# StefanHeng/Symbolic-Music-Generation

Hardware: AMD Instinct MI355X
Metric: train tokens/sec (TransfoXL seq2048 bf16), whole job (higher is better)
Workload: dtype bf16; 1 GPU; TransfoXL 12L/768d H12 dh64 F3072 T=2048 M=2048 V=1190 cutoffs=[] (SURVEY C3, mode R: fresh zero mems); per_gpu_batch=64, global_batch=64, seq_len=2048, mem_len=2048, parallelism=dp1

## Files before the change

### include/musicxl.h

```cpp
#ifndef MUSICXL_H
#define MUSICXL_H

#ifdef __cplusplus
extern "C" {
#endif

#define MXL_ABI_VERSION 2

int mxl_abi_version(void);
const char* mxl_error_string(int code);

#define MXL_GEMM_OUT_F32        0x01
#define MXL_GEMM_OUT_F32_ATOMIC 0x02
#define MXL_GEMM_BIAS           0x04
#define MXL_GEMM_RELU           0x08
#define MXL_GEMM_DROPOUT        0x10
#define MXL_GEMM_RELU_BWD       0x20
#define MXL_GEMM_ADD_AUX        0x40
int mxl_set_reserved_cus(int k);
int mxl_gemm_last_nt_kernel(void);

#define MXL_GEMM_SAVE_RELU_MASK 0x100
#define MXL_GEMM_RELU_BWD_BITS  0x200
size_t mxl_gemm_relu_mask_bytes(int M, int N);
// ... 44 lines not shown
                              long long q_bs, int q_rs, long long kv_bs, int kv_rs, int rd_rs, long long o_bs, int o_rs,
                              long long dq_bs, int dq_rs, long long dkv_bs, int dkv_rs, float scale, void* stream);
int mxl_relattn_fwd_phantom(const void* q, const void* k, const void* v, const void* rd, const float* r_w_bias,
                            const float* r_r_bias, void* out, float* lse, void* oph, float* mph, int B, int T, int H,
                            int dh, int M, int Kc, long long q_bs, int q_rs, long long kv_bs, int kv_rs, int rd_rs,
                            long long o_bs, int o_rs, float scale, void* stream);
int mxl_relattn_bwd_sparse_dg_oph(const void* q, const void* k, const void* v, const void* rd, const float* r_w_bias,
                                  const float* r_r_bias, const void* out, const void* dout, const float* lse,
                                  float* delta, void* dq, void* dk, void* dv, void* dg, float* d_r_w_bias,
                                  const void* oph, const float* mph, int B, int T, int H, int dh, int M, int Kc,
                                  long long q_bs, int q_rs, long long kv_bs, int kv_rs, int rd_rs, long long o_bs, int o_rs,
                                  long long dq_bs, int dq_rs, long long dkv_bs, int dkv_rs, float scale, void* stream);
int mxl_relattn_drd_recompute(const void* dg, const void* qr, float* d_rd, int B, int T, int H, int dh, int M, long long qr_bs,
                              int qr_rs, int drd_ld, const void* rd, int rd_rs, float* d_r_r_bias, float* d_r_w_bias_fix,
                              const float* lse, const float* delta, float scale, int Kc, void* stream);

size_t mxl_relattn_bwd_fused_ws_bytes(int B, int T, int H, int dh, int M);
int mxl_relattn_bwd_fused(const void* q, const void* k, const void* v, const void* rd, const float* r_w_bias,
                          const float* r_r_bias, const void* out, const void* dout, const float* lse, float* delta,
                          void* dq, void* dk, void* dv, float* d_rd, int drd_ld, float* d_r_w_bias, float* d_r_r_bias,
                          const void* oph, const float* mph, void* ws, int B, int T, int H, int dh, int M, int Kc,
                          long long q_bs, int q_rs, long long kv_bs, int kv_rs, int rd_rs, long long o_bs, int o_rs,
                          long long dq_bs, int dq_rs, long long dkv_bs, int dkv_rs, float scale, int defer_finish, void* stream);
int mxl_relattn_dq_finish(const void* ws, const void* oph, const float* mph, const float* lse, const float* delta, void* dq,
                          float* d_r_r_bias, int B, int T, int H, int dh, int M, int Kc, long long o_bs, int o_rs, long long dq_bs,
                          int dq_rs, float scale, void* stream);
int mxl_relattn_fwd_phantom2(const void* q, const void* k, const void* v, const void* rd, const float* r_w_bias,
                             const float* r_r_bias, void* out, float* lse, void* oph, float* mph, int oph_all, void* ph_ws, int B,
                             int T, int H, int dh, int M, int Kc, long long q_bs, int q_rs, long long kv_bs, int kv_rs, int rd_rs,
                             long long o_bs, int o_rs, float scale, void* stream);
size_t mxl_relattn_drd_phantom_ws_bytes(int B, int T, int H);
int mxl_relattn_drd_phantom_prep(const void* q, long long q_bs, int q_rs, const float* r_r_bias, const float* lse, void* ws, int B, int T,
                                 int H, int dh, float scale, void* stream);
int mxl_relattn_drd_phantom(const void* ws, const float* delta, float* d_rd, int B, int T, int H, int dh, int M, int drd_ld,
                            const void* rd, int rd_rs, int Kc, void* stream);

int mxl_sinusoid_table(void* out, int M, int d, int clamp_len, float drop_p, unsigned long long seed, unsigned site,
                       void* stream);
int mxl_embed_fwd(const void* ids, const void* E, void* out, int N, int d, int V, float scale, float drop_p,
                  unsigned long long seed, unsigned site, void* stream);
int mxl_embed_bwd(const void* ids, const void* dout, const void* dout2, float* dE, int N, int d, int V, float scale,
                  float drop_p, unsigned long long seed, unsigned site, void* stream);
int mxl_dropout_bf16(const void* x, void* y, long long n, float drop_p, unsigned long long seed, unsigned site,
                     void* stream);
int mxl_ln_residual_fwd(const void* x, const void* res, const float* gamma, const float* beta, void* y, void* z,
                        float* mean, float* rstd, int N, int d, float eps, float drop_p, unsigned long long seed,
// ... 211 lines not shown
```

### symbolic_music_generation_amd/csrc/musicxl_internal.h

```cpp
#pragma once
#include <hip/hip_runtime.h>
#include "../../include/musicxl.h"

namespace mxl_kt {
extern int g_on;
void begin(int id, hipStream_t s);
void end(int id, hipStream_t s);
struct Scope {
    int id; hipStream_t s; bool on;
    Scope(int id_, hipStream_t s_) : id(id_), s(s_), on(g_on != 0) { if (on) begin(id, s); }
    ~Scope() { if (on) end(id, s); }
};
}
```

### symbolic_music_generation_amd/csrc/relattn_bwd_fused.hip

```cpp
#include <cstdlib>
#include <type_traits>
#include "common.h"
#include "musicxl_internal.h"

namespace {

typedef __attribute__((ext_vector_type(8))) __bf16 mfma_bf16x8;
typedef __attribute__((address_space(3))) bf16x4 lds_bf16x4;
typedef _Float16 f16x4 __attribute__((ext_vector_type(4)));
typedef float f32x4v __attribute__((ext_vector_type(4)));

#ifndef FUSED_PF
#define FUSED_PF 3
#endif
#ifndef FUSED_VF_RELOAD
#define FUSED_VF_RELOAD 0
#endif
#ifndef FUSED_PARK
#define FUSED_PARK 0
#endif
#ifndef FUSED_SB
#define FUSED_SB 1
#endif
#define UNIT_FENCE() do { if (FUSED_SB) __builtin_amdgcn_sched_barrier(0); } while (0)
// ... 37 lines not shown
#define STAMP(i) { unsigned long long t_; __builtin_amdgcn_sched_barrier(0); asm volatile("s_memtime %0\n\ts_waitcnt lgkmcnt(0)" : "=s"(t_) :: "memory"); \
    __builtin_amdgcn_sched_barrier(0); st_acc[i] += t_ - st_last; st_last = t_; }
#define STAMP_FLUSH if ((threadIdx.x & 63) == 0) { for (int i_ = 0; i_ < 16; i_++) atomicAdd(&g_fused_stamps[i_], st_acc[i_]); }
#else
#define STAMP_DECL
#define STAMP(i)
#define STAMP_FLUSH
#endif

#ifndef MXL_SLAB_BF16
#define MXL_SLAB_BF16 1
#endif
#if MXL_SLAB_BF16
typedef bf16_t slab_t;
#else
typedef float slab_t;
#endif

struct FusedP {
    const bf16_t *q, *k, *v, *rd, *dout;
    const float *rwb, *rrb, *lse, *delta;
    bf16_t *dk, *dv;
    slab_t* slab;
    float* drd;
    float *d_rwb, *d_rrb;
    int B, T, H, M, Kc;
    long long q_bs, kv_bs, o_bs, dkv_bs, slab_stride;
    int q_rs, kv_rs, rd_rs, o_rs, dkv_rs, drd_ld;
    float scale, scale_log2e;
};

__device__ __forceinline__ int qswz(int row) { return (((row >> 1) & 1) << 2) | (((row >> 2) & 1) << 1) | ((row >> 3) & 1); }
__device__ __forceinline__ int qoff(int row, int ch) { return row * ROWB + ((ch ^ qswz(row)) << 4); }
__device__ __forceinline__ int qeoff(int row, int e) { return qoff(row, e >> 3) + ((e & 7) << 1); }
__device__ __forceinline__ int sswz(int row) { return (((row >> 3) & 1) << 2) | (((row >> 1) & 1) << 1) | ((row >> 2) & 1); }
__device__ __forceinline__ int soff(int row, int ch) { return row * ROWB + ((ch ^ sswz(row)) << 4); }

__device__ __forceinline__ void lds_barrier() {
    asm volatile("s_waitcnt lgkmcnt(0)" ::: "memory");
    __builtin_amdgcn_s_barrier();
    asm volatile("" ::: "memory");
}

__device__ __forceinline__ uint32_t lds_addr(const void* p) {
    return (uint32_t)(uintptr_t)(__attribute__((address_space(3))) const char*)(const char*)p;
}
// ... 50 lines not shown
__global__ __launch_bounds__(256) void fused_delta_kernel(const bf16_t* o, const bf16_t* dout, float* delta, int B, int T, int H,
                                                          long long o_bs, int o_rs) {
    const int row = blockIdx.x * 4 + (threadIdx.x >> 6);
    if (row >= B * T) return;
    const int lane = threadIdx.x & 63;
    const int b = row / T, i = row % T;
    const bf16_t* op = o + (size_t)b * o_bs + (size_t)i * o_rs;
    const bf16_t* dp = dout + (size_t)b * o_bs + (size_t)i * o_rs;
    const int chunks = H * 8;
    for (int c0 = 0; c0 < chunks; c0 += 64) {
        const int c = c0 + lane;
        float s = 0.f;
        if (c < chunks) {
            const bf16x8 a = *reinterpret_cast<const bf16x8*>(op + c * 8);
            const bf16x8 d = *reinterpret_cast<const bf16x8*>(dp + c * 8);
#pragma unroll
            for (int j = 0; j < 8; j++) s += bf2f((bf16_t)a[j]) * bf2f((bf16_t)d[j]);
        }
        s += __shfl_xor(s, 1, 64); s += __shfl_xor(s, 2, 64); s += __shfl_xor(s, 4, 64);
        if (c < chunks && (lane & 7) == 0) delta[((size_t)b * H + (c >> 3)) * T + i] = s;
    }
}

__global__ __launch_bounds__(512, 1) void relattn_bwd_fused_kernel(FusedP p) {
    constexpr int NT = 512;
    extern __shared__ __attribute__((aligned(16))) char smem[];
    char* sK = smem;
    char* sR = sK + K_BYTES;
    char* sQ = sR + RING_BYTES;
    char* sG = sQ + 2 * QSET;
    char* sX = sG + G_BYTES;
    char* sY = sX + X_BYTES;
    float* sBias = reinterpret_cast<float*>(sY + Y_BYTES);
    float* sPark = sBias + BIAS_BYTES / 4;

    STAMP_DECL
    const int tid = threadIdx.x;
    const int w = __builtin_amdgcn_readfirstlane(tid >> 6);
    const int l = tid & 63, r = l & 31, hh = l >> 5;
    int bx_, h, b;
    xcd_block(bx_, h, b);
    const int T = p.T, M = p.M;
    const int p0 = T - p.Kc;
    const int P0 = p0 + KBLK * bx_;
    const int Pw = P0 + 32 * w;
    const int kloc0 = 32 * w + r;
// ... 6 lines not shown
    const bf16_t* vbase = p.v + (size_t)b * p.kv_bs + (size_t)h * 64;

    const int gq = l >> 4, q4 = (l & 15) >> 2, pp = l & 3;
    int rowq = qoff(r, hh);
    int rows = r * ROWB + ((hh ^ sswz(r)) << 4);
    int tkb = qeoff(4 * hh + q4, 16 * (gq & 1) + 4 * pp);
    const uint32_t gRb = lds_addr(sG) + 4 * hh * (GP + 2) + (256 - kloc0) * 2;
    const uint32_t yWb = lds_addr(sY) + 4 * hh * (YP + 2) + (256 - kloc0) * 2;
    const int xf = (kloc0 >> 1) & 7;
    int xw = kloc0 * 64 + ((((hh ^ (xf & 1)) | (xf & 6))) << 3);
    int yt0 = (4 * (l >> 4) + ((l & 15) >> 2)) * YP + (16 * (w & 1) + 4 * pp) * 2;
    int qb0 = qeoff(4 * (l >> 4) + ((l & 15) >> 2), 16 * (w >> 1) + 4 * pp);
    const int eq = w >> 1, ih0 = w & 1;
    const int g16 = l >> 4, q16 = (l & 15) >> 2;
    int xa0 = ((8 * g16 + q16) * 64 + ((pp ^ ((4 * g16 + (q16 >> 1)) & 7)) << 3)) ^ (ih0 << 5);
    int xa1 = ((8 * g16 + q16 + 4) * 64 + ((pp ^ ((4 * g16 + 2 + (q16 >> 1)) & 7)) << 3)) ^ (ih0 << 5);
    const int kch = 2 * eq + (pp >> 1);
    const int ksw = ((g16 & 1) << 2) | (((q16 >> 1) & 1) << 1);
    int ka0 = (8 * g16 + q16) * ROWB + ((kch ^ ksw) << 4) + ((pp & 1) << 3);
    int ka1 = (8 * g16 + q16 + 4) * ROWB + ((kch ^ (ksw | 1)) << 4) + ((pp & 1) << 3);
    int yq0 = (16 * ih0 + (l & 15)) * YP + 16 * g16;
    int krow = kloc0 * ROWB + ((hh ^ sswz(kloc0)) << 4);

    if (tid < 128) sBias[tid] = (tid < 64) ? p.rwb[h * 64 + tid] : p.rrb[h * 64 + tid - 64];
#pragma unroll
    for (int n = 0; n < 2048 / NT; n++) {
        const int c = tid + n * NT;
        const int row = c >> 3, ch = c & 7;
        const int srow = KBLK * bx_ + row;
        u32x4 val = {0u, 0u, 0u, 0u};
        if (srow < p.Kc) val = *reinterpret_cast<const u32x4*>(kbase + (size_t)srow * p.kv_rs + ch * 8);
        *reinterpret_cast<u32x4*>(sK + soff(row, ch)) = val;
    }
    for (int i = tid; i < Y_BYTES / 16; i += NT) reinterpret_cast<u32x4*>(sY)[i] = u32x4{0u, 0u, 0u, 0u};
    bf16x8 vf[4];
    const bool kok = Pw + r < T;
    {
        const size_t srow = (size_t)(kok ? Pw + r - p0 : 0);
        const bf16_t* vp = vbase + srow * p.kv_rs;
#pragma unroll
        for (int ks = 0; ks < 4; ks++) {
            const bf16x8 vv = *reinterpret_cast<const bf16x8*>(vp + 16 * ks + 8 * hh);
#pragma unroll
            for (int j = 0; j < 8; j++) vf[ks][j] = kok ? vv[j] : (short)0;
        }
    }

    const int i_lo = max(P0, 0), i_hi = min(P0 + KBLK - 1 + M - 1, T - 1);
    const int it_lo = i_lo >> 5, it_hi = i_hi >> 5;

    const bool st_q = w < 4;
    const __amdgpu_buffer_rsrc_t rs_q = __builtin_amdgcn_make_buffer_rsrc((void*)qbase, 0, -1, 0x00020000);
    const __amdgpu_buffer_rsrc_t rs_2 = __builtin_amdgcn_make_buffer_rsrc((void*)(st_q ? rbase : dobase), 0, -1, 0x00020000);
    const __amdgpu_buffer_rsrc_t rs_lse = __builtin_amdgcn_make_buffer_rsrc((void*)(p.lse + ((size_t)b * p.H + h) * T), 0, -1, 0x00020000);
    const __amdgpu_buffer_rsrc_t rs_dl = __builtin_amdgcn_make_buffer_rsrc((void*)(p.delta + ((size_t)b * p.H + h) * T), 0, -1, 0x00020000);
    u32x4 tq = {0u, 0u, 0u, 0u}, t2 = {0u, 0u, 0u, 0u};
    float tl = 0.f, tdl = 0.f;
#define STG_IDS int tid_o = tid; asm volatile("" : "+v"(tid_o)); const int srow_ = (tid_o & 255) >> 3, sch_ = tid_o & 7;
    auto load_stage = [&](int it, int nblk) {
        STG_IDS
        const int I = it * QT;
        tq = __builtin_bit_cast(u32x4, __builtin_amdgcn_raw_buffer_load_b128(rs_q, (srow_ * p.q_rs + sch_ * 8) * 2, I * p.q_rs * 2, 0));
        int d = 32 * nblk + srow_;
        d = d < 0 ? 0 : (d > M - 1 ? M - 1 : d);
        const int vo2 = st_q ? (d * p.rd_rs + sch_ * 8) * 2 : (srow_ * p.o_rs + sch_ * 8) * 2;
        const int so2 = st_q ? 0 : I * p.o_rs * 2;
        t2 = __builtin_bit_cast(u32x4, __builtin_amdgcn_raw_buffer_load_b128(rs_2, vo2, so2, 0));
        tl = __builtin_bit_cast(float, __builtin_amdgcn_raw_buffer_load_b32(rs_lse, (tid & 31) * 4, I * 4, 0));
        tdl = __builtin_bit_cast(float, __builtin_amdgcn_raw_buffer_load_b32(rs_dl, (tid & 31) * 4, I * 4, 0));
    };
    auto store_stage = [&](int buf, int slot) {
        STG_IDS
        char* sQw = sQ + buf * QSET;
        char* sQr = sQw + QIMG;
        char* sDO = sQr + QIMG;
        float* sLse = reinterpret_cast<float*>(sDO + QIMG);
        {
            const bf16_t* src = reinterpret_cast<const bf16_t*>(&tq);
            const float* bb = sBias + (st_q ? 0 : 64) + sch_ * 8;
            const f32x4 b0 = *reinterpret_cast<const f32x4*>(bb), b1 = *reinterpret_cast<const f32x4*>(bb + 4);
            u32x4 wq;
            bf16_t* dq_ = reinterpret_cast<bf16_t*>(&wq);
#pragma unroll
            for (int j = 0; j < 8; j++) dq_[j] = f2bf((bf2f(src[j]) + (j < 4 ? b0[j & 3] : b1[j & 3])) * p.scale_log2e);
            *reinterpret_cast<u32x4*>((st_q ? sQw : sQr) + qoff(srow_, sch_)) = wq;
        }
        if (st_q) {
            *reinterpret_cast<u32x4*>(sR + slot * RBLK_BYTES + soff(srow_, sch_)) = t2;
        } else {
            const bf16_t* src = reinterpret_cast<const bf16_t*>(&t2);
            u32x4 wd;
            bf16_t* dd = reinterpret_cast<bf16_t*>(&wd);
#pragma unroll
            for (int j = 0; j < 8; j++) dd[j] = f2bf(bf2f(src[j]) * p.scale);
            *reinterpret_cast<u32x4*>(sDO + qoff(srow_, sch_)) = wd;
        }
        if (tid < 32) { sLse[tid] = -tl * LOG2E; sLse[QT + tid] = -p.scale * tdl; }
    };
    auto slot_add = [&](int s, int k) { const int x = s + k; return x >= RING_BLKS ? x - RING_BLKS : x; };
    auto gblock = [&](int j, int s0, const bf16x8 (&bq)[4]) {
// ... 548 lines not shown

#ifdef MXL_STAMP
extern "C" int mxl_debug_fused_stamps(unsigned long long* host_out16) {
    hipError_t e = hipMemcpyFromSymbol(host_out16, HIP_SYMBOL(g_fused_stamps), sizeof(unsigned long long) * 16);
    if (e != hipSuccess) return (int)e;
    unsigned long long z[16] = {0};
    e = hipMemcpyToSymbol(HIP_SYMBOL(g_fused_stamps), z, sizeof(z));
    return (int)e;
}
#endif

extern "C" size_t mxl_relattn_bwd_fused_ws_bytes(int B, int T, int H, int dh, int M) {
    if (B <= 0 || T <= 0 || H <= 0 || dh != 64 || M <= 0) return 0;
    return (size_t)((M + KBLK - 1) / KBLK + 1) * (size_t)B * T * H * 64 * sizeof(slab_t);
}

extern "C" int mxl_relattn_bwd_fused(const void* q, const void* k, const void* v, const void* rd, const float* r_w_bias,
                                     const float* r_r_bias, const void* out, const void* dout, const float* lse, float* delta,
                                     void* dq, void* dk, void* dv, float* d_rd, int drd_ld, float* d_r_w_bias, float* d_r_r_bias,
                                     const void* oph, const float* mph, void* ws, int B, int T, int H, int dh, int M, int Kc,
                                     long long q_bs, int q_rs, long long kv_bs, int kv_rs, int rd_rs, long long o_bs, int o_rs,
                                     long long dq_bs, int dq_rs, long long dkv_bs, int dkv_rs, float scale, int defer_finish,
                                     void* stream) {
    MXL_CHECK_ARG(q && k && v && rd && r_w_bias && r_r_bias && out && dout && lse && delta && dq && dk && dv && d_rd && d_r_w_bias &&
                  d_r_r_bias && ws);
    if (dh != 64) return MXL_EUNSUPPORTED;
    MXL_CHECK_ARG(B > 0 && T > 0 && H > 0 && M > 0 && Kc >= T && Kc <= M + T && drd_ld >= H * 64);
    if ((T % 32) != 0 || (M % 32) != 0 || (Kc % 32) != 0) return MXL_EUNSUPPORTED;
    MXL_CHECK_ARG(Kc == M + T || (oph && mph));
    MXL_CHECK_ARG((q_rs % 8) == 0 && (kv_rs % 8) == 0 && (rd_rs % 8) == 0 && (o_rs % 8) == 0 && (dq_rs % 8) == 0 && (dkv_rs % 4) == 0);
    MXL_CHECK_ARG((q_bs % 8) == 0 && (kv_bs % 8) == 0 && (o_bs % 8) == 0 && (dq_bs % 8) == 0 && (dkv_bs % 4) == 0);
    MXL_CHECK_ARG(((uintptr_t)q % 16) == 0 && ((uintptr_t)k % 16) == 0 && ((uintptr_t)v % 16) == 0 && ((uintptr_t)rd % 16) == 0 &&
                  ((uintptr_t)out % 16) == 0 && ((uintptr_t)dout % 16) == 0 && ((uintptr_t)dq % 16) == 0 && ((uintptr_t)ws % 16) == 0 &&
                  (oph == nullptr || ((uintptr_t)oph % 16) == 0));
    hipStream_t s = (hipStream_t)stream;
    static bool attr_set = false;
    if (!attr_set) {
        hipError_t e = hipFuncSetAttribute(reinterpret_cast<const void*>(&relattn_bwd_fused_kernel), hipFuncAttributeMaxDynamicSharedMemorySize, SMEM);
        if (e != hipSuccess) return (int)e;
        attr_set = true;
    }
    const bool delta_ready = (defer_finish & 2) != 0;
    defer_finish &= 1;
    if (!delta_ready) {
        mxl_kt::Scope kt(MXL_KT_RELATTN_DELTA, s);
        hipLaunchKernelGGL(fused_delta_kernel, dim3((B * T + 3) / 4), dim3(256), 0, s, (const bf16_t*)out, (const bf16_t*)dout, delta, B, T,
                           H, o_bs, o_rs);
    }
    FusedP p;
    p.q = (const bf16_t*)q; p.k = (const bf16_t*)k; p.v = (const bf16_t*)v; p.rd = (const bf16_t*)rd; p.dout = (const bf16_t*)dout;
    p.rwb = r_w_bias; p.rrb = r_r_bias; p.lse = lse; p.delta = delta;
    p.dk = (bf16_t*)dk; p.dv = (bf16_t*)dv; p.slab = (slab_t*)ws; p.drd = d_rd; p.d_rwb = d_r_w_bias; p.d_rrb = d_r_r_bias;
    p.B = B; p.T = T; p.H = H; p.M = M; p.Kc = Kc;
    p.q_bs = q_bs; p.kv_bs = kv_bs; p.o_bs = o_bs; p.dkv_bs = dkv_bs; p.slab_stride = (long long)B * T * H * 64;
    p.q_rs = q_rs; p.kv_rs = kv_rs; p.rd_rs = rd_rs; p.o_rs = o_rs; p.dkv_rs = dkv_rs; p.drd_ld = drd_ld;
    p.scale = scale; p.scale_log2e = scale * LOG2E;
    {
        mxl_kt::Scope kt(MXL_KT_RELATTN_FUSED, s);
        hipLaunchKernelGGL(relattn_bwd_fused_kernel, dim3((Kc + KBLK - 1) / KBLK, H, B), dim3(512), SMEM, s, p);
    }
    MXL_LAUNCH_CHECK();
    if (defer_finish) return MXL_OK;
    return mxl_relattn_dq_finish(ws, oph, mph, lse, delta, dq, d_r_r_bias, B, T, H, dh, M, Kc, o_bs, o_rs, dq_bs, dq_rs, scale, stream);
}

extern "C" int mxl_relattn_dq_finish(const void* ws, const void* oph, const float* mph, const float* lse, const float* delta, void* dq,
                                     float* d_r_r_bias, int B, int T, int H, int dh, int M, int Kc, long long o_bs, int o_rs,
                                     long long dq_bs, int dq_rs, float scale, void* stream) {
    MXL_CHECK_ARG(ws && lse && delta && dq && B > 0 && T > 0 && H > 0 && M > 0 && Kc >= T && Kc <= M + T);
    if (dh != 64 || (T % 32) != 0 || (M % 32) != 0 || (Kc % 32) != 0) return MXL_EUNSUPPORTED;
    MXL_CHECK_ARG(Kc == M + T || (oph && mph));
    MXL_CHECK_ARG((o_rs % 8) == 0 && (o_bs % 8) == 0 && (dq_rs % 8) == 0 && (dq_bs % 8) == 0 && ((uintptr_t)dq % 16) == 0 &&
                  ((uintptr_t)ws % 16) == 0 && (oph == nullptr || ((uintptr_t)oph % 16) == 0));
    hipStream_t s = (hipStream_t)stream;
    FinP f;
    f.slab = (const slab_t*)ws; f.oph = (Kc < M + T) ? (const bf16_t*)oph : nullptr; f.mph = mph; f.lse = lse; f.delta = delta;
    f.dq = (bf16_t*)dq; f.d_rrb = d_r_r_bias;
    f.B = B; f.T = T; f.H = H; f.M = M; f.Kc = Kc;
    f.slab_stride = (long long)B * T * H * 64; f.o_bs = o_bs; f.dq_bs = dq_bs; f.o_rs = o_rs; f.dq_rs = dq_rs; f.scale = scale;
    {
        mxl_kt::Scope kt(MXL_KT_RELATTN_DQFIN, s);
        const long long rgs = (long long)B * (T / FIN_ROWS);
// ... 9 lines not shown
```

### symbolic_music_generation_amd/csrc/relattn_drd_phantom.hip

```cpp
#include "common.h"
#include "musicxl_internal.h"

namespace {

typedef __attribute__((ext_vector_type(8))) __bf16 mfma_bf16x8;
typedef __attribute__((address_space(3))) void* lptr_t;
constexpr float LOG2E = 1.4426950408889634f;

__device__ __forceinline__ float mul1(float a, float b) {
    float r;
    asm("v_mul_f32 %0, %1, %2" : "=v"(r) : "v"(a), "v"(b));
    return r;
}
__device__ __forceinline__ f32x16 mfma32(bf16x8 a, bf16x8 b, f32x16 c) {
    return __builtin_amdgcn_mfma_f32_32x32x16_bf16(__builtin_bit_cast(mfma_bf16x8, a), __builtin_bit_cast(mfma_bf16x8, b), c, 0, 0, 0);
}
typedef unsigned long long u64x2 __attribute__((ext_vector_type(2)));
__device__ __forceinline__ void tr_read8(uint32_t a0, uint32_t a1, bf16x8 (&fb)[2][2]) {
    u64x2 v00, v01, v10, v11;
    asm volatile(
        "ds_read_b64_tr_b16 %0, %8\n\tds_read_b64_tr_b16 %1, %9 offset:1024\n\t"
        "ds_read_b64_tr_b16 %2, %8 offset:2048\n\tds_read_b64_tr_b16 %3, %9 offset:3072\n\t"
        "ds_read_b64_tr_b16 %4, %10\n\tds_read_b64_tr_b16 %5, %11 offset:1024\n\t"
        "ds_read_b64_tr_b16 %6, %10 offset:2048\n\tds_read_b64_tr_b16 %7, %11 offset:3072\n\t"
        "s_waitcnt lgkmcnt(0)"
        : "=&v"(v00.x), "=&v"(v00.y), "=&v"(v01.x), "=&v"(v01.y), "=&v"(v10.x), "=&v"(v10.y), "=&v"(v11.x), "=&v"(v11.y)
        : "v"(a0), "v"(a0 ^ 16u), "v"(a1), "v"(a1 ^ 16u)
        : "memory");
    fb[0][0] = __builtin_bit_cast(bf16x8, v00); fb[0][1] = __builtin_bit_cast(bf16x8, v01);
    fb[1][0] = __builtin_bit_cast(bf16x8, v10); fb[1][1] = __builtin_bit_cast(bf16x8, v11);
}

constexpr int PH_REC = 4096 + 256;
__device__ __forceinline__ int ph_swz(int row) { return (((row >> 1) & 1) << 2) | (((row >> 2) & 1) << 1) | ((row >> 3) & 1); }

__global__ void phantom_prep_kernel(const bf16_t* q, long long q_bs, int q_rs, const float* rrb, char* rec, int B, int T, int H,
                                    float scale_log2e) {
    const int chunks = H * 8;
    const long long gid = (long long)blockIdx.x * blockDim.x + threadIdx.x;
    if (gid >= (long long)B * T * chunks) return;
    const int c = (int)(gid % chunks);
    const long long row = gid / chunks;
    const int b = (int)(row / T), t = (int)(row % T);
    const bf16x8 v = *reinterpret_cast<const bf16x8*>(q + b * q_bs + (long long)t * q_rs + c * 8);
    float o[8];
#pragma unroll
    for (int j = 0; j < 8; j++) o[j] = (bf2f((bf16_t)v[j]) + rrb[c * 8 + j]) * scale_log2e;
    const u32x4 w = {pack2bf(o[0], o[1]), pack2bf(o[2], o[3]), pack2bf(o[4], o[5]), pack2bf(o[6], o[7])};
    const int r = t & 31;
    char* dst = rec + (((size_t)b * H + (c >> 3)) * (T >> 5) + (t >> 5)) * PH_REC + r * 128 + (((c & 7) ^ ph_swz(r)) << 4);
    *reinterpret_cast<u32x4*>(dst) = w;
}
__global__ void phantom_prep_sc_kernel(const float* lse, char* rec, long long n, int T) {
    const long long i = (long long)blockIdx.x * blockDim.x + threadIdx.x;
    if (i >= n) return;
    const long long bh = i / T;
// ... 212 lines not shown
    STAMP_FLUSH
}

}

#ifdef MXL_STAMP
extern "C" int mxl_debug_phantom_occupancy() {
    int n = -1;
    hipFuncSetAttribute(reinterpret_cast<const void*>(&relattn_drd_phantom_kernel), hipFuncAttributeMaxDynamicSharedMemorySize, PH_SMEM);
    hipError_t e = hipOccupancyMaxActiveBlocksPerMultiprocessor(&n, relattn_drd_phantom_kernel, 256, PH_SMEM);
    return e == hipSuccess ? n : -(int)e;
}
extern "C" int mxl_debug_phantom_stamps(unsigned long long* host_out16) {
    hipError_t e = hipMemcpyFromSymbol(host_out16, HIP_SYMBOL(g_ph_stamps), sizeof(unsigned long long) * 16);
    if (e != hipSuccess) return (int)e;
    unsigned long long z[16] = {0};
    e = hipMemcpyToSymbol(HIP_SYMBOL(g_ph_stamps), z, sizeof(z));
    return (int)e;
}
#endif

extern "C" size_t mxl_relattn_drd_phantom_ws_bytes(int B, int T, int H) {
    if (B <= 0 || T <= 0 || H <= 0 || (T % 32) != 0) return 0;
    return (size_t)B * H * (T / 32) * PH_REC;
}

extern "C" int mxl_relattn_drd_phantom_prep(const void* q, long long q_bs, int q_rs, const float* r_r_bias, const float* lse, void* ws,
                                            int B, int T, int H, int dh, float scale, void* stream) {
    MXL_CHECK_ARG(q && r_r_bias && lse && ws && B > 0 && T > 0 && H > 0);
    if (dh != 64 || (T % 32) != 0) return MXL_EUNSUPPORTED;
    MXL_CHECK_ARG((q_rs % 8) == 0 && (q_bs % 8) == 0 && ((uintptr_t)q % 16) == 0 && ((uintptr_t)ws % 16) == 0);
    const long long tot = (long long)B * T * (H * 8), nsc = (long long)B * H * T;
    {
        mxl_kt::Scope kt(MXL_KT_ROWBIAS, (hipStream_t)stream);
        hipLaunchKernelGGL(phantom_prep_kernel, dim3((unsigned)((tot + 255) / 256)), dim3(256), 0, (hipStream_t)stream, (const bf16_t*)q,
                           q_bs, q_rs, r_r_bias, (char*)ws, B, T, H, scale * LOG2E);
        hipLaunchKernelGGL(phantom_prep_sc_kernel, dim3((unsigned)((nsc + 255) / 256)), dim3(256), 0, (hipStream_t)stream, lse,
                           (char*)ws, nsc, T);
    }
    MXL_LAUNCH_CHECK();
    return MXL_OK;
}

extern "C" int mxl_relattn_drd_phantom(const void* ws, const float* delta, float* d_rd, int B, int T, int H, int dh, int M, int drd_ld,
                                       const void* rd, int rd_rs, int Kc, void* stream) {
    MXL_CHECK_ARG(ws && delta && d_rd && rd && B > 0 && T > 0 && H > 0 && M > 0 && Kc >= T && Kc <= M + T);
    if (dh != 64 || (T % 32) != 0 || (M % 32) != 0 || (M + 255) / 256 > 32) return MXL_EUNSUPPORTED;
// ... 44 lines not shown
```

### symbolic_music_generation_amd/csrc/relattn_fwd.hip

```cpp
#include <type_traits>
#include "common.h"
#include "musicxl_internal.h"

namespace {

typedef __attribute__((ext_vector_type(8))) __bf16 mfma_bf16x8;
typedef __attribute__((address_space(3))) bf16x4 lds_bf16x4;

struct RelAttnP {
    const bf16_t *q, *k, *v, *rd;
    const float *rwb, *rrb;
    bf16_t* out;
    float* lse;
    int B, T, H, M, Kc;
    long long q_bs, kv_bs, o_bs;
    int q_rs, kv_rs, rd_rs, o_rs;
    float scale_log2e;
    bf16_t* oph;
    float* mph;
    int oph_all;
    char* ph_rec;
};

constexpr int QB = 128;
// ... 118 lines not shown
    const bf16_t* kbase = p.k + (size_t)b * p.kv_bs + (size_t)h * DH;
    const bf16_t* vbase = p.v + (size_t)b * p.kv_bs + (size_t)h * DH;
    const bf16_t* rbase = p.rd + (size_t)h * DH;

    bf16x8 qw[KS], qr[KS];
    {
        const int i = iw0 + r;
        const bool ok = i < T;
        const bf16_t* qp = p.q + (size_t)b * p.q_bs + (size_t)(ok ? i : 0) * p.q_rs + (size_t)h * DH;
#pragma unroll
        for (int ks = 0; ks < KS; ks++) {
            const int e0 = 16 * ks + 8 * hh;
            bf16x8 qv = *reinterpret_cast<const bf16x8*>(qp + e0);
#pragma unroll
            for (int j = 0; j < 8; j++) {
                const float qf = ok ? bf2f((bf16_t)qv[j]) : 0.f;
                qw[ks][j] = (short)f2bf((qf + p.rwb[h * DH + e0 + j]) * p.scale_log2e);
                qr[ks][j] = (short)f2bf((qf + p.rrb[h * DH + e0 + j]) * p.scale_log2e);
            }
        }
    }

    if (p.ph_rec && iw0 < T) {
        char* rec = p.ph_rec + (((size_t)b * p.H + h) * (size_t)(T >> 5) + (iw0 >> 5)) * 4352;
        const int sw = (((r >> 1) & 1) << 2) | (((r >> 2) & 1) << 1) | ((r >> 3) & 1);
#pragma unroll
        for (int ks = 0; ks < KS; ks++) *reinterpret_cast<bf16x8*>(rec + r * 128 + (((2 * ks + hh) ^ sw) << 4)) = qr[ks];
    }

    const int p_lo = i0 - M + 1;
    const int p_hi = min(i0 + QB - 1, T - 1);
    const int kt_lo = floordiv(p_lo, KT), kt_hi = floordiv(p_hi, KT);

    typedef u32x4 stage_t[G::NLD_K];
    stage_t rk, rv, rr[2];
    const unsigned kv_bytes = (unsigned)(((long long)(p.Kc - 1) * p.kv_rs + DH) * 2);
    const unsigned rd_bytes = (unsigned)(((long long)(M - 1) * p.rd_rs + DH) * 2);
    const __amdgpu_buffer_rsrc_t rs_k = __builtin_amdgcn_make_buffer_rsrc((void*)kbase, 0, (int)kv_bytes, 0x00020000);
    const __amdgpu_buffer_rsrc_t rs_v = __builtin_amdgcn_make_buffer_rsrc((void*)vbase, 0, (int)kv_bytes, 0x00020000);
    const __amdgpu_buffer_rsrc_t rs_r = __builtin_amdgcn_make_buffer_rsrc((void*)rbase, 0, (int)rd_bytes, 0x00020000);
    constexpr bool STG_ALL = (KT * G::CH) % 256 == 0;
    int kvo[G::NLD_K], rdo[G::NLD_K], kst[G::NLD_K], vst[G::NLD_K];
#pragma unroll
    for (int n = 0; n < G::NLD_K; n++) {
        const int c = tid + n * 256;
        const int row = c / G::CH, ch = c % G::CH;
        kvo[n] = ((row - p0) * p.kv_rs + ch * 8) * 2;
        rdo[n] = (row * p.rd_rs + ch * 8) * 2;
        kst[n] = G::koff(row & (KT - 1), ch);
        vst[n] = G::voff(row & (KT - 1), ch * 16);
// ... 427 lines not shown
    }
    STAMP(15)

    const float l_tot = l_run + __shfl_xor(l_run, 32, 64);
    const float inv = l_tot > 0.f ? 1.f / l_tot : 0.f;
    const int qi = iw0 + r;
    if (qi < T) {
        bf16_t* op = p.out + (size_t)b * p.o_bs + (size_t)qi * p.o_rs + (size_t)h * DH;
#pragma unroll
        for (int e = 0; e < EB; e++) {
#pragma unroll
            for (int grp = 0; grp < 4; grp++) {
                const int e0 = 32 * e + 8 * grp + 4 * hh;
                if (e0 < DH) {
                    u32x2 w = {pack2bf(o[e][4 * grp] * inv, o[e][4 * grp + 1] * inv),
                               pack2bf(o[e][4 * grp + 2] * inv, o[e][4 * grp + 3] * inv)};
                    *reinterpret_cast<u32x2*>(op + e0) = w;
                }
            }
        }
        const float lse2 = m_run + __builtin_amdgcn_logf(l_tot);
        if (hh == 0 && p.lse) p.lse[((size_t)b * p.H + h) * T + qi] = lse2 * 0.6931471805599453f;
        if (hh == 0 && p.ph_rec)
            reinterpret_cast<float*>(p.ph_rec + (((size_t)b * p.H + h) * (size_t)(T >> 5) + (iw0 >> 5)) * 4352 + 4096)[r] = -lse2;
    }
    STAMP(15)
    STAMP_FLUSH
}

template <int DH>
int launch_fwd(const RelAttnP& p, hipStream_t s) {
    using G = Geo<DH>;
    static bool attr_set = false;
    if (!attr_set) {
        hipError_t e = hipFuncSetAttribute(reinterpret_cast<const void*>(&relattn_fwd_kernel<DH>),
                                           hipFuncAttributeMaxDynamicSharedMemorySize, G::SMEM);
        if (e != hipSuccess) return (int)e;
        attr_set = true;
    }
    dim3 grid((p.T + QB - 1) / QB, p.H, p.B);
    {
        mxl_kt::Scope kt(MXL_KT_RELATTN_FWD, s);
        hipLaunchKernelGGL((relattn_fwd_kernel<DH>), grid, dim3(256), G::SMEM, s, p);
    }
    MXL_LAUNCH_CHECK();
    return MXL_OK;
}
// ... 69 lines not shown
```

### symbolic_music_generation_amd/ops.py

```python
import ctypes as C
import math
import os
from typing import Optional, Sequence

import torch

from ._lib import lib, check, MusicXLError

GEMM_OUT_F32 = 0x01
GEMM_OUT_F32_ATOMIC = 0x02
GEMM_BIAS = 0x04
GEMM_RELU = 0x08
GEMM_DROPOUT = 0x10
GEMM_RELU_BWD = 0x20
GEMM_ADD_AUX = 0x40
GEMM_SAVE_RELU_MASK = 0x100
GEMM_RELU_BWD_BITS = 0x200


def mix_seed(base_seed: int, step: int) -> int:
    import torch.distributed as dist
    rank = dist.get_rank() if (dist.is_available() and dist.is_initialized()) else 0
    x = (base_seed * 0x9E3779B97F4A7C15 + rank * 0xD1B54A32D192ED03 + step * 0x2545F4914F6CDD1D) & 0xFFFFFFFFFFFFFFFF
    x ^= x >> 32
# ... 643 lines not shown

_PH_WS = {}


def _phantom_ws(B, T, H, device):
    key = (B, T, H, str(device))
    buf = _PH_WS.get(key)
    if buf is None:
        buf = torch.empty(int(lib().mxl_relattn_drd_phantom_ws_bytes(B, T, H)), device=device, dtype=torch.uint8)
        _PH_WS[key] = buf
    return buf


def gemm_headdot(a, b, c, M, N, K, o, T, delta, lda=None, ldb=None, ldc=None, ldo=None):
    rc = lib().mxl_gemm_bf16_headdot(_p(a), _p(b), _p(c), M, N, K, lda or K, ldb or K, ldc or N, _p(o), ldo or N, T, _p(delta), _stream())
    if rc == -2:
        return False
    check(rc, 'mxl_gemm_bf16_headdot')
    return True


def relattn_bwd_fused(q, k, v, rd, r_w_bias, r_r_bias, out, dout, lse, delta, dq, dk, dv, d_rd, d_rwb, d_rrb, ws, qr_buf, *,
                      B, T, H, dh, M, Kc, q_bs, q_rs, kv_bs, kv_rs, rd_rs, o_bs, o_rs, dq_bs, dq_rs, dkv_bs, dkv_rs,
                      scale=None, oph=None, mph=None, defer_drd=False, ph_buf=None, ph_ready=False, delta_ready=False):
    scale = scale if scale is not None else 1.0 / math.sqrt(dh)
    d = H * dh
    check(lib().mxl_relattn_bwd_fused(_p(q), _p(k), _p(v), _p(rd), _p(r_w_bias), _p(r_r_bias), _p(out), _p(dout), _p(lse), _p(delta),
                                      _p(dq), _p(dk), _p(dv), _p(d_rd), d_rd.stride(0), _p(d_rwb), _p(d_rrb), _p(oph), _p(mph), _p(ws),
                                      B, T, H, dh, M, Kc, q_bs, q_rs, kv_bs, kv_rs, rd_rs, o_bs, o_rs, dq_bs, dq_rs, dkv_bs, dkv_rs,
                                      float(scale), 2 if delta_ready else 0, _stream()), 'mxl_relattn_bwd_fused')

    def phantom():
        if Kc < M + T:
            ph = ph_buf if ph_buf is not None else _phantom_ws(B, T, H, q.device)
            if not (ph_ready and ph_buf is not None):
                check(lib().mxl_relattn_drd_phantom_prep(_p(q), q_bs, q_rs, _p(r_r_bias), _p(lse), _p(ph), B, T, H, dh, float(scale),
                                                         _stream()), 'mxl_relattn_drd_phantom_prep')
            check(lib().mxl_relattn_drd_phantom(_p(ph), _p(delta), _p(d_rd), B, T, H, dh, M, d_rd.stride(0), _p(rd), int(rd_rs), Kc,
                                                _stream()), 'mxl_relattn_drd_phantom')
    if defer_drd:
        return phantom
    phantom()
    return None


def relattn_drd(q, r_r_bias, dg, d_rd, qr_buf, *, B, T, H, dh, M, q_bs, q_rs, rd=None, rd_rs=0, d_rrb=None, d_rwb=None,
                recompute=None):
    d = H * dh
    add_rowbias(q, q_bs, q_rs, r_r_bias.reshape(-1), qr_buf, B, T, d)
    if recompute is not None:
        check(lib().mxl_relattn_drd_recompute(_p(dg), _p(qr_buf), _p(d_rd), B, T, H, dh, M, T * d, d, d, _p(rd), int(rd_rs),
                                              _p(d_rrb), _p(d_rwb), _p(recompute['lse']), _p(recompute['delta']),
                                              float(recompute['scale']), int(recompute['Kc']), _stream()),
# ... 206 lines not shown
```

Measured before the change: 856,300 tokens/s.

## Reuse forward-pass biased Q records in fused attention backward instead of recomputing

The forward kernel now also writes the r_w_bias-added, swizzled q tile (qw) next to the existing qr phantom records. A templated backward kernel variant loads these pre-biased, pre-swizzled tiles straight into shared memory, skipping the strided q load, the bias add and the swizzle per stage. This removes backward arithmetic and address work, but costs extra forward writes and doubles the phantom workspace size. It is only used when the phantom records are ready and Kc < M+T.

```diff
diff --git a/include/musicxl.h b/include/musicxl.h
--- a/include/musicxl.h
+++ b/include/musicxl.h
@@ -90,6 +90,12 @@
                           const void* oph, const float* mph, void* ws, int B, int T, int H, int dh, int M, int Kc,
                           long long q_bs, int q_rs, long long kv_bs, int kv_rs, int rd_rs, long long o_bs, int o_rs,
                           long long dq_bs, int dq_rs, long long dkv_bs, int dkv_rs, float scale, int defer_finish, void* stream);
+int mxl_relattn_bwd_fused_rec(const void* q, const void* k, const void* v, const void* rd, const float* r_w_bias,
+                              const float* r_r_bias, const void* out, const void* dout, const float* lse, float* delta,
+                              void* dq, void* dk, void* dv, float* d_rd, int drd_ld, float* d_r_w_bias, float* d_r_r_bias,
+                              const void* oph, const float* mph, void* ws, const void* ph_rec, int B, int T, int H, int dh, int M,
+                              int Kc, long long q_bs, int q_rs, long long kv_bs, int kv_rs, int rd_rs, long long o_bs, int o_rs,
+                              long long dq_bs, int dq_rs, long long dkv_bs, int dkv_rs, float scale, int defer_finish, void* stream);
 int mxl_relattn_dq_finish(const void* ws, const void* oph, const float* mph, const float* lse, const float* delta, void* dq,
                           float* d_r_r_bias, int B, int T, int H, int dh, int M, int Kc, long long o_bs, int o_rs, long long dq_bs,
                           int dq_rs, float scale, void* stream);
diff --git a/symbolic_music_generation_amd/csrc/musicxl_internal.h b/symbolic_music_generation_amd/csrc/musicxl_internal.h
--- a/symbolic_music_generation_amd/csrc/musicxl_internal.h
+++ b/symbolic_music_generation_amd/csrc/musicxl_internal.h
@@ -1,6 +1,9 @@
 #pragma once
 #include <hip/hip_runtime.h>
 #include "../../include/musicxl.h"
+
+constexpr int MXL_PH_REC = 4096 + 256;
+constexpr int MXL_QW_REC = MXL_PH_REC;
 
 namespace mxl_kt {
 extern int g_on;
diff --git a/symbolic_music_generation_amd/csrc/relattn_bwd_fused.hip b/symbolic_music_generation_amd/csrc/relattn_bwd_fused.hip
--- a/symbolic_music_generation_amd/csrc/relattn_bwd_fused.hip
+++ b/symbolic_music_generation_amd/csrc/relattn_bwd_fused.hip
@@ -83,6 +83,7 @@
     const float *rwb, *rrb, *lse, *delta;
     bf16_t *dk, *dv;
     slab_t* slab;
+    const char* rec;
     float* drd;
     float *d_rwb, *d_rrb;
     int B, T, H, M, Kc;
@@ -179,6 +180,7 @@
     }
 }
 
+template <bool REC>
 __global__ __launch_bounds__(512, 1) void relattn_bwd_fused_kernel(FusedP p) {
     constexpr int NT = 512;
     extern __shared__ __attribute__((aligned(16))) char smem[];
@@ -231,7 +233,7 @@
     int yq0 = (16 * ih0 + (l & 15)) * YP + 16 * g16;
     int krow = kloc0 * ROWB + ((hh ^ sswz(kloc0)) << 4);
 
-    if (tid < 128) sBias[tid] = (tid < 64) ? p.rwb[h * 64 + tid] : p.rrb[h * 64 + tid - 64];
+    if (!REC && tid < 128) sBias[tid] = (tid < 64) ? p.rwb[h * 64 + tid] : p.rrb[h * 64 + tid - 64];
 #pragma unroll
     for (int n = 0; n < 2048 / NT; n++) {
         const int c = tid + n * NT;
@@ -259,7 +261,11 @@
     const int it_lo = i_lo >> 5, it_hi = i_hi >> 5;
 
     const bool st_q = w < 4;
-    const __amdgpu_buffer_rsrc_t rs_q = __builtin_amdgcn_make_buffer_rsrc((void*)qbase, 0, -1, 0x00020000);
+    const size_t rec_tiles = ((size_t)b * p.H + h) * (size_t)(T >> 5);
+    const char* recbase = REC ? p.rec + (st_q ? (size_t)p.B * p.H * (size_t)(T >> 5) * MXL_PH_REC + rec_tiles * MXL_QW_REC : rec_tiles * MXL_PH_REC)
+                              : nullptr;
+    const int rec_stride = st_q ? MXL_QW_REC : MXL_PH_REC;
+    const __amdgpu_buffer_rsrc_t rs_q = __builtin_amdgcn_make_buffer_rsrc(REC ? (void*)recbase : (void*)qbase, 0, -1, 0x00020000);
     const __amdgpu_buffer_rsrc_t rs_2 = __builtin_amdgcn_make_buffer_rsrc((void*)(st_q ? rbase : dobase), 0, -1, 0x00020000);
     const __amdgpu_buffer_rsrc_t rs_lse = __builtin_amdgcn_make_buffer_rsrc((void*)(p.lse + ((size_t)b * p.H + h) * T), 0, -1, 0x00020000);
     const __amdgpu_buffer_rsrc_t rs_dl = __builtin_amdgcn_make_buffer_rsrc((void*)(p.delta + ((size_t)b * p.H + h) * T), 0, -1, 0x00020000);
@@ -269,7 +275,8 @@
     auto load_stage = [&](int it, int nblk) {
         STG_IDS
         const int I = it * QT;
-        tq = __builtin_bit_cast(u32x4, __builtin_amdgcn_raw_buffer_load_b128(rs_q, (srow_ * p.q_rs + sch_ * 8) * 2, I * p.q_rs * 2, 0));
+        if (REC) tq = __builtin_bit_cast(u32x4, __builtin_amdgcn_raw_buffer_load_b128(rs_q, (tid_o & 255) * 16, it * rec_stride, 0));
+        else tq = __builtin_bit_cast(u32x4, __builtin_amdgcn_raw_buffer_load_b128(rs_q, (srow_ * p.q_rs + sch_ * 8) * 2, I * p.q_rs * 2, 0));
         int d = 32 * nblk + srow_;
         d = d < 0 ? 0 : (d > M - 1 ? M - 1 : d);
         const int vo2 = st_q ? (d * p.rd_rs + sch_ * 8) * 2 : (srow_ * p.o_rs + sch_ * 8) * 2;
@@ -284,7 +291,9 @@
         char* sQr = sQw + QIMG;
         char* sDO = sQr + QIMG;
         float* sLse = reinterpret_cast<float*>(sDO + QIMG);
-        {
+        if (REC) {
+            *reinterpret_cast<u32x4*>((st_q ? sQw : sQr) + (tid_o & 255) * 16) = tq;
+        } else {
             const bf16_t* src = reinterpret_cast<const bf16_t*>(&tq);
             const float* bb = sBias + (st_q ? 0 : 64) + sch_ * 8;
             const f32x4 b0 = *reinterpret_cast<const f32x4*>(bb), b1 = *reinterpret_cast<const f32x4*>(bb + 4);
@@ -879,6 +888,18 @@
                                      long long q_bs, int q_rs, long long kv_bs, int kv_rs, int rd_rs, long long o_bs, int o_rs,
                                      long long dq_bs, int dq_rs, long long dkv_bs, int dkv_rs, float scale, int defer_finish,
                                      void* stream) {
+    return mxl_relattn_bwd_fused_rec(q, k, v, rd, r_w_bias, r_r_bias, out, dout, lse, delta, dq, dk, dv, d_rd, drd_ld, d_r_w_bias, d_r_r_bias,
+                                     oph, mph, ws, nullptr, B, T, H, dh, M, Kc, q_bs, q_rs, kv_bs, kv_rs, rd_rs, o_bs, o_rs, dq_bs, dq_rs,
+                                     dkv_bs, dkv_rs, scale, defer_finish, stream);
+}
+
+extern "C" int mxl_relattn_bwd_fused_rec(const void* q, const void* k, const void* v, const void* rd, const float* r_w_bias,
+                                         const float* r_r_bias, const void* out, const void* dout, const float* lse, float* delta,
+                                         void* dq, void* dk, void* dv, float* d_rd, int drd_ld, float* d_r_w_bias, float* d_r_r_bias,
+                                         const void* oph, const float* mph, void* ws, const void* ph_rec, int B, int T, int H, int dh,
+                                         int M, int Kc, long long q_bs, int q_rs, long long kv_bs, int kv_rs, int rd_rs, long long o_bs,
+                                         int o_rs, long long dq_bs, int dq_rs, long long dkv_bs, int dkv_rs, float scale,
+                                         int defer_finish, void* stream) {
     MXL_CHECK_ARG(q && k && v && rd && r_w_bias && r_r_bias && out && dout && lse && delta && dq && dk && dv && d_rd && d_r_w_bias &&
                   d_r_r_bias && ws);
     if (dh != 64) return MXL_EUNSUPPORTED;
@@ -889,11 +910,14 @@
     MXL_CHECK_ARG((q_bs % 8) == 0 && (kv_bs % 8) == 0 && (o_bs % 8) == 0 && (dq_bs % 8) == 0 && (dkv_bs % 4) == 0);
     MXL_CHECK_ARG(((uintptr_t)q % 16) == 0 && ((uintptr_t)k % 16) == 0 && ((uintptr_t)v % 16) == 0 && ((uintptr_t)rd % 16) == 0 &&
                   ((uintptr_t)out % 16) == 0 && ((uintptr_t)dout % 16) == 0 && ((uintptr_t)dq % 16) == 0 && ((uintptr_t)ws % 16) == 0 &&
-                  (oph == nullptr || ((uintptr_t)oph % 16) == 0));
+                  (oph == nullptr || ((uintptr_t)oph % 16) == 0) && ((uintptr_t)ph_rec % 16) == 0);
+    MXL_CHECK_ARG(ph_rec == nullptr || (long long)(T / 32) * MXL_PH_REC < (1ll << 31));
     hipStream_t s = (hipStream_t)stream;
     static bool attr_set = false;
     if (!attr_set) {
-        hipError_t e = hipFuncSetAttribute(reinterpret_cast<const void*>(&relattn_bwd_fused_kernel), hipFuncAttributeMaxDynamicSharedMemorySize, SMEM);
+        hipError_t e = hipFuncSetAttribute(reinterpret_cast<const void*>(&relattn_bwd_fused_kernel<false>), hipFuncAttributeMaxDynamicSharedMemorySize, SMEM);
+        if (e == hipSuccess)
+            e = hipFuncSetAttribute(reinterpret_cast<const void*>(&relattn_bwd_fused_kernel<true>), hipFuncAttributeMaxDynamicSharedMemorySize, SMEM);
         if (e != hipSuccess) return (int)e;
         attr_set = true;
     }
@@ -907,6 +931,7 @@
     FusedP p;
     p.q = (const bf16_t*)q; p.k = (const bf16_t*)k; p.v = (const bf16_t*)v; p.rd = (const bf16_t*)rd; p.dout = (const bf16_t*)dout;
     p.rwb = r_w_bias; p.rrb = r_r_bias; p.lse = lse; p.delta = delta;
+    p.rec = (const char*)ph_rec;
     p.dk = (bf16_t*)dk; p.dv = (bf16_t*)dv; p.slab = (slab_t*)ws; p.drd = d_rd; p.d_rwb = d_r_w_bias; p.d_rrb = d_r_r_bias;
     p.B = B; p.T = T; p.H = H; p.M = M; p.Kc = Kc;
     p.q_bs = q_bs; p.kv_bs = kv_bs; p.o_bs = o_bs; p.dkv_bs = dkv_bs; p.slab_stride = (long long)B * T * H * 64;
@@ -914,7 +939,9 @@
     p.scale = scale; p.scale_log2e = scale * LOG2E;
     {
         mxl_kt::Scope kt(MXL_KT_RELATTN_FUSED, s);
-        hipLaunchKernelGGL(relattn_bwd_fused_kernel, dim3((Kc + KBLK - 1) / KBLK, H, B), dim3(512), SMEM, s, p);
+        const dim3 grid((Kc + KBLK - 1) / KBLK, H, B);
+        if (ph_rec) hipLaunchKernelGGL(relattn_bwd_fused_kernel<true>, grid, dim3(512), SMEM, s, p);
+        else hipLaunchKernelGGL(relattn_bwd_fused_kernel<false>, grid, dim3(512), SMEM, s, p);
     }
     MXL_LAUNCH_CHECK();
     if (defer_finish) return MXL_OK;
diff --git a/symbolic_music_generation_amd/csrc/relattn_drd_phantom.hip b/symbolic_music_generation_amd/csrc/relattn_drd_phantom.hip
--- a/symbolic_music_generation_amd/csrc/relattn_drd_phantom.hip
+++ b/symbolic_music_generation_amd/csrc/relattn_drd_phantom.hip
@@ -31,7 +31,7 @@
     fb[1][0] = __builtin_bit_cast(bf16x8, v10); fb[1][1] = __builtin_bit_cast(bf16x8, v11);
 }
 
-constexpr int PH_REC = 4096 + 256;
+constexpr int PH_REC = MXL_PH_REC;
 __device__ __forceinline__ int ph_swz(int row) { return (((row >> 1) & 1) << 2) | (((row >> 2) & 1) << 1) | ((row >> 3) & 1); }
 
 __global__ void phantom_prep_kernel(const bf16_t* q, long long q_bs, int q_rs, const float* rrb, char* rec, int B, int T, int H,
@@ -290,7 +290,7 @@
 
 extern "C" size_t mxl_relattn_drd_phantom_ws_bytes(int B, int T, int H) {
     if (B <= 0 || T <= 0 || H <= 0 || (T % 32) != 0) return 0;
-    return (size_t)B * H * (T / 32) * PH_REC;
+    return (size_t)B * H * (T / 32) * (PH_REC + MXL_QW_REC);
 }
 
 extern "C" int mxl_relattn_drd_phantom_prep(const void* q, long long q_bs, int q_rs, const float* r_r_bias, const float* lse, void* ws,
diff --git a/symbolic_music_generation_amd/csrc/relattn_fwd.hip b/symbolic_music_generation_amd/csrc/relattn_fwd.hip
--- a/symbolic_music_generation_amd/csrc/relattn_fwd.hip
+++ b/symbolic_music_generation_amd/csrc/relattn_fwd.hip
@@ -164,10 +164,15 @@
     }
 
     if (p.ph_rec && iw0 < T) {
-        char* rec = p.ph_rec + (((size_t)b * p.H + h) * (size_t)(T >> 5) + (iw0 >> 5)) * 4352;
+        const size_t tix = ((size_t)b * p.H + h) * (size_t)(T >> 5) + (iw0 >> 5);
+        char* rec = p.ph_rec + tix * MXL_PH_REC;
+        char* recw = p.ph_rec + (size_t)p.B * p.H * (size_t)(T >> 5) * MXL_PH_REC + tix * MXL_QW_REC;
         const int sw = (((r >> 1) & 1) << 2) | (((r >> 2) & 1) << 1) | ((r >> 3) & 1);
 #pragma unroll
-        for (int ks = 0; ks < KS; ks++) *reinterpret_cast<bf16x8*>(rec + r * 128 + (((2 * ks + hh) ^ sw) << 4)) = qr[ks];
+        for (int ks = 0; ks < KS; ks++) {
+            *reinterpret_cast<bf16x8*>(rec + r * 128 + (((2 * ks + hh) ^ sw) << 4)) = qr[ks];
+            *reinterpret_cast<bf16x8*>(recw + r * 128 + (((2 * ks + hh) ^ sw) << 4)) = qw[ks];
+        }
     }
 
     const int p_lo = i0 - M + 1;
@@ -641,7 +646,7 @@
         const float lse2 = m_run + __builtin_amdgcn_logf(l_tot);
         if (hh == 0 && p.lse) p.lse[((size_t)b * p.H + h) * T + qi] = lse2 * 0.6931471805599453f;
         if (hh == 0 && p.ph_rec)
-            reinterpret_cast<float*>(p.ph_rec + (((size_t)b * p.H + h) * (size_t)(T >> 5) + (iw0 >> 5)) * 4352 + 4096)[r] = -lse2;
+            reinterpret_cast<float*>(p.ph_rec + (((size_t)b * p.H + h) * (size_t)(T >> 5) + (iw0 >> 5)) * MXL_PH_REC + 4096)[r] = -lse2;
     }
     STAMP(15)
     STAMP_FLUSH
diff --git a/symbolic_music_generation_amd/ops.py b/symbolic_music_generation_amd/ops.py
--- a/symbolic_music_generation_amd/ops.py
+++ b/symbolic_music_generation_amd/ops.py
@@ -689,13 +689,17 @@
 
 def relattn_bwd_fused(q, k, v, rd, r_w_bias, r_r_bias, out, dout, lse, delta, dq, dk, dv, d_rd, d_rwb, d_rrb, ws, qr_buf, *,
                       B, T, H, dh, M, Kc, q_bs, q_rs, kv_bs, kv_rs, rd_rs, o_bs, o_rs, dq_bs, dq_rs, dkv_bs, dkv_rs,
-                      scale=None, oph=None, mph=None, defer_drd=False, ph_buf=None, ph_ready=False, delta_ready=False):
+                      scale=None, oph=None, mph=None, defer_drd=False, ph_buf=None, ph_ready=False, delta_ready=False,
+                      use_records=True):
     scale = scale if scale is not None else 1.0 / math.sqrt(dh)
     d = H * dh
-    check(lib().mxl_relattn_bwd_fused(_p(q), _p(k), _p(v), _p(rd), _p(r_w_bias), _p(r_r_bias), _p(out), _p(dout), _p(lse), _p(delta),
-                                      _p(dq), _p(dk), _p(dv), _p(d_rd), d_rd.stride(0), _p(d_rwb), _p(d_rrb), _p(oph), _p(mph), _p(ws),
-                                      B, T, H, dh, M, Kc, q_bs, q_rs, kv_bs, kv_rs, rd_rs, o_bs, o_rs, dq_bs, dq_rs, dkv_bs, dkv_rs,
-                                      float(scale), 2 if delta_ready else 0, _stream()), 'mxl_relattn_bwd_fused')
+    rec = ph_buf if (use_records and ph_ready and ph_buf is not None and Kc < M + T
+                     and os.environ.get('MXL_FUSED_NO_RECORDS') != '1') else None
+    check(lib().mxl_relattn_bwd_fused_rec(_p(q), _p(k), _p(v), _p(rd), _p(r_w_bias), _p(r_r_bias), _p(out), _p(dout), _p(lse), _p(delta),
+                                          _p(dq), _p(dk), _p(dv), _p(d_rd), d_rd.stride(0), _p(d_rwb), _p(d_rrb), _p(oph), _p(mph),
+                                          _p(ws), _p(rec), B, T, H, dh, M, Kc, q_bs, q_rs, kv_bs, kv_rs, rd_rs, o_bs, o_rs, dq_bs,
+                                          dq_rs, dkv_bs, dkv_rs, float(scale), 2 if delta_ready else 0, _stream()),
+          'mxl_relattn_bwd_fused_rec')
 
     def phantom():
         if Kc < M + T:
```

After: 841,200 tokens/s. 0.982x the previous value.
